# yezhen17/3DIoUMatch

Measured on AMD Instinct MI355X. Metric: scenes/sec train-step (ScanNet 40k pts, 256 proposals), higher is better.
Workload: dtype f32; 1 GPU; ScanNet pretrain step (BASELINE configs[1]): VoteNet-IoU forward_with_pred_jitter + labeled loss + backward + Adam; per_gpu_batch=8, global_batch=8, num_points=40000, num_proposals=256, parallelism=dp1, fps_prefetch_one_step_ahead=True, hip_graphs=True

## Files before the change

3dioumatch_amd/csrc/mlp_gemm.hip:

```cpp
#include "common.h"
#include "mlp_operand.h"
#include <mutex>
#include <stdlib.h>

namespace {

constexpr int KC = 16;

template <int TM, int TN, int WM, int WN, int MODE, bool A_TRANS>
__global__ void __launch_bounds__(256)
gemm_nn_kernel(int m_total, int k_total, int r, const float *__restrict__ a, int lda, OperandB opb,
               float *__restrict__ c, size_t b_stride_in, size_t b_stride_out) {
  constexpr int MB = TM / WM / 32, NB = TN / WN / 32;
  constexpr int LDA = TM + 4;
  __shared__ float As[KC * LDA];
  __shared__ __attribute__((aligned(16))) float Bs[KC * TN];
  const int tid = threadIdx.x, lane = tid & 63, wave = tid >> 6;
  const int wm = wave / WN, wn = wave % WN;
  const int r0 = blockIdx.x * TN, m0 = blockIdx.y * TM, b = blockIdx.z;
  OperandB op = opb;
  const size_t in_off = (size_t)b * b_stride_in;

  f32x16 acc[MB][NB];
#pragma unroll
  for (int i = 0; i < MB; ++i)
#pragma unroll
    for (int j = 0; j < NB; ++j)
#pragma unroll
      for (int q = 0; q < 16; ++q) acc[i][j][q] = 0.f;

  constexpr int AE = TM * KC / 256;
  constexpr int SEG = TN / 16;
  const int bkk = tid >> 4, bnn = (tid & 15) * SEG;
  const bool vec_ok = (r & 3) == 0;
  float areg[AE], bx[SEG], bdz[SEG];
  RowCoef rc;
  bool brow_ok = false;
  auto fetch = [&](int k0) {
#pragma unroll
    for (int e = 0; e < AE; ++e) {
      const int t = tid + e * 256;
      const int kk = A_TRANS ? t / TM : t % KC, mm = A_TRANS ? t % TM : t / KC;
      const int gm = m0 + mm, gk = k0 + kk;
      const size_t at = A_TRANS ? (size_t)gk * lda + gm : (size_t)gm * lda + gk;
      areg[e] = (gm < m_total && gk < k_total) ? a[at] : 0.f;
    }
    const int gk = k0 + bkk;
    brow_ok = gk < k_total;
    rc = load_row_coef<MODE>(op, gk, brow_ok);
    load_raw_segment<MODE, SEG>(op, in_off + (size_t)gk * r + r0 + bnn, r0 + bnn, r, vec_ok,
                                brow_ok, bx, bdz, b * k_total + gk);
  };
  auto stash = [&]() {
#pragma unroll
    for (int e = 0; e < AE; ++e) {
      const int t = tid + e * 256;
      As[(A_TRANS ? t / TM : t % KC) * LDA + (A_TRANS ? t % TM : t / KC)] = areg[e];
    }
#pragma unroll
    for (int i = 0; i < SEG; i += 4) {
      float4 v;
      v.x = (brow_ok && r0 + bnn + i + 0 < r) ? transform<MODE>(bx[i + 0], bdz[i + 0], rc) : 0.f;
      v.y = (brow_ok && r0 + bnn + i + 1 < r) ? transform<MODE>(bx[i + 1], bdz[i + 1], rc) : 0.f;
      v.z = (brow_ok && r0 + bnn + i + 2 < r) ? transform<MODE>(bx[i + 2], bdz[i + 2], rc) : 0.f;
      v.w = (brow_ok && r0 + bnn + i + 3 < r) ? transform<MODE>(bx[i + 3], bdz[i + 3], rc) : 0.f;
      *reinterpret_cast<float4 *>(&Bs[bkk * TN + bnn + i]) = v;
    }
  };
  fetch(0);
  for (int k0 = 0; k0 < k_total; k0 += KC) {
    __syncthreads();
    stash();
    __syncthreads();
    if (k0 + KC < k_total) fetch(k0 + KC);
#pragma unroll
    for (int kk = 0; kk < KC; kk += 2) {
      const int krow = kk + (lane >> 5);
      float af[MB], bf[NB];
#pragma unroll
      for (int i = 0; i < MB; ++i) af[i] = As[krow * LDA + (wm * MB + i) * 32 + (lane & 31)];
#pragma unroll
      for (int j = 0; j < NB; ++j) bf[j] = Bs[krow * TN + (wn * NB + j) * 32 + (lane & 31)];
#pragma unroll
      for (int i = 0; i < MB; ++i)
#pragma unroll
        for (int j = 0; j < NB; ++j)
          acc[i][j] = __builtin_amdgcn_mfma_f32_32x32x2f32(af[i], bf[j], acc[i][j], 0, 0, 0);
    }
// ... 299 lines not shown
    constexpr int GPL = 32 / (PL < 32 ? PL : 32);
#pragma unroll
    for (int i = 0; i < MB; ++i) {
      const int rbase = m0 + (wm * MB + i) * 32;
#pragma unroll
      for (int q = 0; q < 16; ++q) {
        const int cq = (q & 3) + 8 * (q >> 2);
        const int rowq = rbase + cq + 4 * half;
        const bool neg = POOL != 0 && rowq < m_total && pool_gamma[rowq] < 0.f;
        const int rsw = (cq & 15) ^ (half << 2);
#pragma unroll
        for (int j = 0; j < NB; ++j) {
          const int col = j * 32 + l31;
          const float v = acc[i][j][q];
          park[(cq + 4 * half) * 64 + ((((col >> 2) ^ rsw) << 2) | (col & 3))] = neg ? -v : v;
        }
      }
      float best[GPL];
      int at[GPL];
#pragma unroll
      for (int gq = 0; gq < GPL; ++gq) { best[gq] = -__builtin_inff(); at[gq] = 0; }
      const float4 *prow = reinterpret_cast<const float4 *>(park + l31 * 64);
      float t1 = 0.f, t2 = 0.f, tsh = 0.f;
#pragma unroll
      for (int c4 = 0; c4 < 8; ++c4) {
        const float4 v4 = prow[(half * 8 + c4) ^ (l31 & 15)];
        const float vv[4] = {v4.x, v4.y, v4.z, v4.w};
        if (SCAN_STATS && c4 == 0) tsh = vv[0];
#pragma unroll
        for (int e = 0; e < 4; ++e) {
          if constexpr (POOL != 0) {
            const int s2 = c4 * 4 + e;
            const int gq = GPL == 2 ? s2 / 16 : 0;
            if (vv[e] > best[gq]) { best[gq] = vv[e]; at[gq] = GPL == 2 ? s2 % 16 : s2; }
          }
          if constexpr (SCAN_STATS) {
            const float d = vv[e] - tsh;
            t1 += d;
            t2 = __fmaf_rn(d, d, t2);
          }
        }
      }
      if constexpr (SCAN_STATS) {
        const float mh = tsh + t1 * (1.0f / 32.0f), qh = fmaxf(t2 - t1 * t1 * (1.0f / 32.0f), 0.f);
        const float mo = __shfl_xor(mh, 32, kWave), qo = __shfl_xor(qh, 32, kWave);
        if (half == 0) {
          const float dlt = mo - mh;
          float mean = 0.5f * (mh + mo);
          const float m2w = (qh + qo) + 16.0f * dlt * dlt;
          if (POOL != 0 && rbase + l31 < m_total && pool_gamma[rbase + l31] < 0.f) mean = -mean;
          wave_stat[wn][(wm * MB + i) * 32 + l31] = make_float2(mean, m2w);
        }
      }
      if (POOL == 64) {
        const float ob = __shfl_xor(best[0], 32, kWave);
        const int oa = __shfl_xor(at[0], 32, kWave);
        if (half == 0 && ob > best[0]) { best[0] = ob; at[0] = 32 + oa; }
      }
      const int row = rbase + l31;
      if (POOL != 0 && row < m_total && (POOL != 64 || half == 0)) {
        const bool negr = pool_gamma[row] < 0.f;
        const int g0 = (r0 + wn * 64) / POOL + (POOL == 64 ? 0 : half * GPL);
        int *ei = reinterpret_cast<int *>(ext);
#pragma unroll
        for (int gq = 0; gq < GPL; ++gq) {
          const size_t o = ((size_t)b * m_total + row) * groups + g0 + gq;
          ext[o] = negr ? -best[gq] : best[gq];
          ei[ext_plane + o] = at[gq];
        }
      }
    }
    if constexpr (SCAN_STATS) merge_wave_stats();
  }
}

constexpr int KS = 64;

struct AImage {
  const unsigned short *p;
  int pitch;
  size_t plane;
};

template <int MODE, bool A_TRANS, bool X6, bool AIMG = false>
__device__ __forceinline__ void gemm_nn_small_body(int blk_x, int blk_y, int blk_z, int m_total, int k_total,
                                                   int r, const float *__restrict__ a, int lda,
                                                   OperandB opb, float *__restrict__ c,
                                                   size_t b_stride_in, size_t b_stride_out,
                                                   const AImage img = AImage{nullptr, 0, 0}) {
  constexpr int TM = 64, TN = 64, LDA = TM + 1;
  constexpr int STAGE = KS * LDA + KS * TN, REDUCE = 4 * 16 * 64;
  __shared__ __attribute__((aligned(16))) float lds[STAGE > REDUCE ? STAGE : REDUCE];
  float *As = lds + KS * TN, *Bs = lds;
  const int tid = threadIdx.x, lane = tid & 63, wave = tid >> 6;
  const int r0 = blk_x * TN, m0 = blk_y * TM, b = blk_z;
  OperandB op = opb;
  const size_t in_off = (size_t)b * b_stride_in;
  f32x16 acc[2][2];
#pragma unroll
  for (int i = 0; i < 2; ++i)
#pragma unroll
    for (int j = 0; j < 2; ++j)
#pragma unroll
      for (int q = 0; q < 16; ++q) acc[i][j][q] = 0.f;

  const int bkk = tid >> 2, bnn = (tid & 3) * 16;
  const bool vec_ok = (r & 3) == 0;
  float areg[16], bx[16], bdz[16];
  RowCoef rc;
  bool brow_ok = false;
  static_assert(!AIMG || X6, "images feed the bf16 form only");
  const bf16x8 *img8 = reinterpret_cast<const bf16x8 *>(img.p);
  auto fetch = [&](int k0) {
    if constexpr (!AIMG) {
#pragma unroll
      for (int e = 0; e < 16; ++e) {
        const int t = tid + e * 256;
        const int kk = A_TRANS ? t / TM : t % KS, mm = A_TRANS ? t % TM : t / KS;
        const int gm = m0 + mm, gk = k0 + kk;
        const size_t at = A_TRANS ? (size_t)gk * lda + gm : (size_t)gm * lda + gk;
        areg[e] = (gm < m_total && gk < k_total) ? a[at] : 0.f;
      }
    }
    const int gk = k0 + bkk;
    brow_ok = gk < k_total;
    rc = load_row_coef<MODE>(op, gk, brow_ok);
    load_raw_segment<MODE, 16>(op, in_off + (size_t)gk * r + r0 + bnn, r0 + bnn, r, vec_ok,
                               brow_ok, bx, bdz, b * k_total + gk);
  };
  fetch(0);
  for (int k0 = 0; k0 < k_total; k0 += KS) {
    Split3 sa_img[2];
    if constexpr (AIMG) {
      const int k0w = wave * (KS / 4) + 8 * (lane >> 5);
#pragma unroll
      for (int i = 0; i < 2; ++i) {
        const size_t at = ((size_t)(m0 + i * 32 + (lane & 31)) * img.pitch + k0 + k0w) >> 3;
        sa_img[i].hi = img8[at];
        sa_img[i].mid = img8[at + (img.plane >> 3)];
        sa_img[i].lo = img8[at + 2 * (img.plane >> 3)];
      }
    }
    __syncthreads();
    if constexpr (!AIMG) {
#pragma unroll
      for (int e = 0; e < 16; ++e) {
        const int t = tid + e * 256;
        As[(A_TRANS ? t / TM : t % KS) * LDA + (A_TRANS ? t % TM : t / KS)] = areg[e];
      }
    }
#pragma unroll
    for (int i = 0; i < 16; i += 4) {
      float4 v;
      v.x = (brow_ok && r0 + bnn + i + 0 < r) ? transform<MODE>(bx[i + 0], bdz[i + 0], rc) : 0.f;
      v.y = (brow_ok && r0 + bnn + i + 1 < r) ? transform<MODE>(bx[i + 1], bdz[i + 1], rc) : 0.f;
      v.z = (brow_ok && r0 + bnn + i + 2 < r) ? transform<MODE>(bx[i + 2], bdz[i + 2], rc) : 0.f;
      v.w = (brow_ok && r0 + bnn + i + 3 < r) ? transform<MODE>(bx[i + 3], bdz[i + 3], rc) : 0.f;
      *reinterpret_cast<float4 *>(&Bs[bkk * TN + bnn + i]) = v;
    }
    __syncthreads();
    if (k0 + KS < k_total) fetch(k0 + KS);
    if constexpr (X6) {
      static_assert(KS / 4 == 16, "a wave's share of the chunk is one 16-deep MFMA step");
      const int k0w = wave * (KS / 4) + 8 * (lane >> 5);
      Split3 sa[2], sb[2];
      if constexpr (AIMG) {
        sa[0] = sa_img[0]; sa[1] = sa_img[1];
      } else {
#pragma unroll
        for (int i = 0; i < 2; ++i) {
          float v[8];
#pragma unroll
          for (int e = 0; e < 8; ++e) v[e] = As[(k0w + e) * LDA + i * 32 + (lane & 31)];
          sa[i] = split3(v);
        }
      }
#pragma unroll
      for (int j = 0; j < 2; ++j) {
        float v[8];
#pragma unroll
        for (int e = 0; e < 8; ++e) v[e] = Bs[(k0w + e) * TN + j * 32 + (lane & 31)];
        sb[j] = split3(v);
      }
#pragma unroll
      for (int i = 0; i < 2; ++i)
#pragma unroll
        for (int j = 0; j < 2; ++j) mfma_x6(acc[i][j], sa[i], sb[j]);
    } else {
#pragma unroll
    for (int kk = 0; kk < KS / 4; kk += 2) {
      const int krow = wave * (KS / 4) + kk + (lane >> 5);
      float af[2], bf[2];
#pragma unroll
      for (int i = 0; i < 2; ++i) af[i] = As[krow * LDA + i * 32 + (lane & 31)];
#pragma unroll
      for (int j = 0; j < 2; ++j) bf[j] = Bs[krow * TN + j * 32 + (lane & 31)];
#pragma unroll
      for (int i = 0; i < 2; ++i)
#pragma unroll
        for (int j = 0; j < 2; ++j)
          acc[i][j] = __builtin_amdgcn_mfma_f32_32x32x2f32(af[i], bf[j], acc[i][j], 0, 0, 0);
    }
    }
  }
  for (int s = 1; s < 4; ++s) {
    __syncthreads();
    if (wave == s) {
#pragma unroll
      for (int i = 0; i < 2; ++i)
#pragma unroll
        for (int j = 0; j < 2; ++j)
#pragma unroll
          for (int q = 0; q < 16; ++q) lds[((i * 2 + j) * 16 + q) * 64 + lane] = acc[i][j][q];
    }
    __syncthreads();
    if (wave == 0) {
#pragma unroll
      for (int i = 0; i < 2; ++i)
#pragma unroll
        for (int j = 0; j < 2; ++j)
#pragma unroll
          for (int q = 0; q < 16; ++q) acc[i][j][q] += lds[((i * 2 + j) * 16 + q) * 64 + lane];
    }
  }
  if (wave != 0) return;
  float *cb = c + (size_t)b * b_stride_out;
#pragma unroll
  for (int i = 0; i < 2; ++i)
#pragma unroll
    for (int j = 0; j < 2; ++j) {
      const int col = r0 + j * 32 + (lane & 31);
#pragma unroll
      for (int q = 0; q < 16; ++q) {
        const int row = m0 + i * 32 + (q & 3) + 8 * (q >> 2) + 4 * (lane >> 5);
        if (row < m_total && col < r) __builtin_nontemporal_store(acc[i][j][q], &cb[(size_t)row * r + col]);
      }
    }
}

template <int MODE, bool A_TRANS, bool X6 = false, bool AIMG = false>
__global__ void __launch_bounds__(256, (X6 && A_TRANS) ? 2 : 1)
gemm_nn_small_kernel(int m_total, int k_total, int r, const float *__restrict__ a, int lda,
                     OperandB opb, float *__restrict__ c, size_t b_stride_in,
                     size_t b_stride_out, AImage img) {
  gemm_nn_small_body<MODE, A_TRANS, X6, AIMG>((int)blockIdx.x, (int)blockIdx.y, (int)blockIdx.z, m_total,
                                              k_total, r, a, lda, opb, c, b_stride_in, b_stride_out, img);
}

constexpr int RC = 32;

template <int PMODE, int QMODE, int KBW, int WK, int RS>
__global__ void __launch_bounds__(256)
gemm_wgrad_kernel(int m_total, int k_begin, int k_end, int k_total, int r, int r_per_slice,
                  OperandB opp, OperandB opq, float *__restrict__ part, size_t p_stride,
                  size_t q_stride) {
  static_assert(WK * RS == 4, "four waves");
  constexpr int TM = 64, TK = 32 * KBW * WK;
  constexpr int QSEG = TK / 64;
  constexpr int LDP = TM + 1, LDQ = TK + 1;
  constexpr int STAGE = RC * (LDP + LDQ);
  constexpr int REDUCE = RS > 1 ? WK * 2 * KBW * 16 * 64 : 0;
  __shared__ float lds[STAGE > REDUCE ? STAGE : REDUCE];
  float *Ps = lds, *Qs = lds + RC * LDP;
  const int tid = threadIdx.x, lane = tid & 63, wave = tid >> 6;
  const int wk = wave % WK, wr = wave / WK;
  const BlockId blk = xcd_block_id();
  const int k0 = k_begin + blk.x * TK, m0 = blk.y * TM;
  const int slices = (r + r_per_slice - 1) / r_per_slice;
  const int b = blk.z / slices, slice = blk.z % slices;
  const int r_lo = slice * r_per_slice;
  const int r_hi = r_lo + r_per_slice < r ? r_lo + r_per_slice : r;
  OperandB P = opp, Q = opq;
  const size_t p_off = (size_t)b * p_stride, q_off = (size_t)b * q_stride;

  f32x16 acc[2][KBW];
#pragma unroll
  for (int i = 0; i < 2; ++i)
#pragma unroll
    for (int j = 0; j < KBW; ++j)
#pragma unroll
      for (int q = 0; q < 16; ++q) acc[i][j][q] = 0.f;

  const int seg_row = tid >> 2, seg_r = (tid & 3) * 8;
  const bool p_ok = m0 + seg_row < m_total;
  const RowCoef pc = load_row_coef<PMODE>(P, m0 + seg_row, p_ok);
  const size_t p_row = p_off + (size_t)(m0 + seg_row) * r;
  bool q_ok[QSEG];
  RowCoef qc[QSEG];
  size_t q_row[QSEG];
#pragma unroll
  for (int s = 0; s < QSEG; ++s) {
    const int gk = k0 + seg_row + 64 * s;
    q_ok[s] = gk < k_end;
    qc[s] = load_row_coef<QMODE>(Q, gk, q_ok[s]);
    q_row[s] = q_off + (size_t)gk * r;
  }
  const bool vec_ok = ((r | r_hi) & 3) == 0;
  float px[8], pdz[8], qx[QSEG][8], qdz[QSEG][8];
  auto fetch = [&](int rr) {
    load_raw_segment<PMODE, 8>(P, p_row + rr + seg_r, rr + seg_r, r_hi, vec_ok, p_ok, px, pdz,
                               b * m_total + m0 + seg_row);
#pragma unroll
    for (int s = 0; s < QSEG; ++s)
      load_raw_segment<QMODE, 8>(Q, q_row[s] + rr + seg_r, rr + seg_r, r_hi, vec_ok, q_ok[s],
                                 qx[s], qdz[s]);
  };
  fetch(r_lo);
  for (int rr = r_lo; rr < r_hi; rr += RC) {
    __syncthreads();
#pragma unroll
    for (int i = 0; i < 8; ++i)
      Ps[(seg_r + i) * LDP + seg_row] =
          (p_ok && rr + seg_r + i < r_hi) ? transform<PMODE>(px[i], pdz[i], pc) : 0.f;
#pragma unroll
    for (int s = 0; s < QSEG; ++s)
#pragma unroll
      for (int i = 0; i < 8; ++i)
        Qs[(seg_r + i) * LDQ + seg_row + 64 * s] =
            (q_ok[s] && rr + seg_r + i < r_hi) ? transform<QMODE>(qx[s][i], qdz[s][i], qc[s]) : 0.f;
    __syncthreads();
    if (rr + RC < r_hi) fetch(rr + RC);
#pragma unroll
    for (int st = 0; st < RC / 2 / RS; ++st) {
      const int row = wr * (RC / RS) + 2 * st + (lane >> 5);
      float bq[KBW], ap[2];
#pragma unroll
      for (int j = 0; j < KBW; ++j) bq[j] = Qs[row * LDQ + (wk * KBW + j) * 32 + (lane & 31)];
#pragma unroll
// ... 73 lines not shown
    q_ok[i] = gk < k_total;
    pc[i] = load_row_coef<PMODE>(P, gm, p_ok[i]);
    qc[i] = load_row_coef<QMODE>(Q, gk, q_ok[i]);
    p_row[i] = (size_t)b * p_stride + (size_t)gm * r;
    q_row[i] = (size_t)b * q_stride + (size_t)gk * r;
  }
  const bool vec_ok = (r & 3) == 0;
  float px[2][16], pdz[2][16], qx[2][16], qdz[2][16];
  auto fetch = [&](int c0) {
    const int col = c0 + 16 * half;
#pragma unroll
    for (int i = 0; i < 2; ++i) {
      load_raw_segment<PMODE, 16>(P, p_row[i] + col, col, r_hi, vec_ok, p_ok[i], px[i], pdz[i]);
      load_raw_segment<QMODE, 16>(Q, q_row[i] + col, col, r_hi, vec_ok, q_ok[i], qx[i], qdz[i]);
    }
  };
  int c0 = r_lo + 32 * wave;
  if (c0 < r_hi) fetch(c0);
  for (; c0 < r_hi; c0 += 128) {
    const int col = c0 + 16 * half;
#pragma unroll
    for (int st = 0; st < 2; ++st) {
      Split3 sp[2], sq[2];
#pragma unroll
      for (int i = 0; i < 2; ++i) {
        float vp[8], vq[8];
#pragma unroll
        for (int e = 0; e < 8; ++e) {
          const bool in = col + 8 * st + e < r_hi;
          vp[e] = (p_ok[i] && in) ? transform<PMODE>(px[i][8 * st + e], pdz[i][8 * st + e], pc[i]) : 0.f;
          vq[e] = (q_ok[i] && in) ? transform<QMODE>(qx[i][8 * st + e], qdz[i][8 * st + e], qc[i]) : 0.f;
        }
        sp[i] = split3(vp);
        sq[i] = split3(vq);
      }
      if (st == 1 && c0 + 128 < r_hi) fetch(c0 + 128);
#pragma unroll
      for (int i = 0; i < 2; ++i)
#pragma unroll
        for (int j = 0; j < 2; ++j) mfma_x6(acc[i][j], sp[i], sq[j]);
    }
  }
#pragma unroll
  for (int i = 0; i < 2; ++i)
#pragma unroll
    for (int j = 0; j < 2; ++j) {
      __syncthreads();
      if (wave != 0) {
#pragma unroll
        for (int q = 0; q < 16; ++q) red[((wave * 16) + q) * 64 + lane] = acc[i][j][q];
      }
      __syncthreads();
      if (wave == 0) {
#pragma unroll
        for (int q = 0; q < 16; ++q)
          acc[i][j][q] += (red[(16 + q) * 64 + lane] + red[(32 + q) * 64 + lane]) + red[(48 + q) * 64 + lane];
      }
    }
  if (wave != 0) return;
  float *out = part + (size_t)blk.z * m_total * k_total;
#pragma unroll
  for (int i = 0; i < 2; ++i)
#pragma unroll
    for (int j = 0; j < 2; ++j) {
      const int col = k0 + j * 32 + l31;
#pragma unroll
      for (int q = 0; q < 16; ++q) {
        const int row = m0 + i * 32 + (q & 3) + 8 * (q >> 2) + 4 * half;
        if (row < m_total && col < k_total) out[(size_t)row * k_total + col] = acc[i][j][q];
      }
    }
}

template <int PMODE, int QMODE>
__global__ void __launch_bounds__(256, 2)
gemm_wgrad_direct_kernel(int m_total, int k_total, int r, int r_per_slice, int slices, OperandB opp,
                         OperandB opq, float *__restrict__ part, size_t p_stride, size_t q_stride) {
  wgrad_direct_body<PMODE, QMODE>(xcd_block_id(), m_total, k_total, r, r_per_slice, slices, opp, opq,
                                  part, p_stride, q_stride);
}

struct SmallPairArgs {
  int nd, dgx, dgy;
  int m, k, r;
  int wkx, wmy, per, slices;
  const float *w;
  float *dq, *part;
  AImage wt_img;
};

template <int PMODE, int QMODE, bool X6D, bool AIMG = false>
__global__ void __launch_bounds__(256, 2)
gemm_small_backward_pair_kernel(SmallPairArgs t, OperandB opp, OperandB opq) {
  const int id = (int)blockIdx.x;
  if (id < t.nd) {
    const int bx = id % t.dgx, by = (id / t.dgx) % t.dgy, bz = id / (t.dgx * t.dgy);
    gemm_nn_small_body<PMODE, true, X6D, AIMG>(bx, by, bz, t.k, t.m, t.r, t.w, t.k, opp, t.dq,
                                               (size_t)t.m * t.r, (size_t)t.k * t.r, t.wt_img);
  } else {
    const int wid = id - t.nd;
    BlockId blk;
    blk.x = wid % t.wkx;
    blk.y = (wid / t.wkx) % t.wmy;
    blk.z = wid / (t.wkx * t.wmy);
    wgrad_direct_body<PMODE, QMODE>(blk, t.m, t.k, t.r, t.per, t.slices, opp, opq, t.part,
                                    (size_t)t.m * t.r, (size_t)t.k * t.r);
  }
}

template <bool VEC>
__device__ __forceinline__ void reduce_partials_block(int block, int count, int parts,
                                                      const float *__restrict__ part,
                                                      float *__restrict__ out) {
  constexpr int W = VEC ? 4 : 1;
  __shared__ float sums[8][32 * W];
  const int e = threadIdx.x & 31, grp = threadIdx.x >> 5;
  const int i = (block * 32 + e) * W;
  float s[8][W];
#pragma unroll
  for (int u = 0; u < 8; ++u)
#pragma unroll
    for (int c = 0; c < W; ++c) s[u][c] = 0.f;
  auto row = [&](int p, float (&v)[W]) {
    if constexpr (VEC) {
      const float4 t = *reinterpret_cast<const float4 *>(part + (size_t)p * count + i);
      v[0] = t.x; v[1] = t.y; v[2] = t.z; v[3] = t.w;
    } else {
      v[0] = part[(size_t)p * count + i];
    }
  };
  if (i < count) {
    int p = grp;
    for (; p + 56 < parts; p += 64) {
      float v[8][W];
#pragma unroll
      for (int u = 0; u < 8; ++u) row(p + 8 * u, v[u]);
#pragma unroll
      for (int u = 0; u < 8; ++u)
#pragma unroll
        for (int c = 0; c < W; ++c) s[u][c] += v[u][c];
    }
    for (; p + 24 < parts; p += 32) {
      float v[4][W];
#pragma unroll
      for (int u = 0; u < 4; ++u) row(p + 8 * u, v[u]);
#pragma unroll
      for (int u = 0; u < 4; ++u)
#pragma unroll
        for (int c = 0; c < W; ++c) s[u][c] += v[u][c];
    }
    for (; p < parts; p += 8) {
      float v[W];
      row(p, v);
#pragma unroll
      for (int c = 0; c < W; ++c) s[0][c] += v[c];
    }
  }
#pragma unroll
  for (int c = 0; c < W; ++c)
    sums[grp][e * W + c] = ((s[0][c] + s[1][c]) + (s[2][c] + s[3][c])) + ((s[4][c] + s[5][c]) + (s[6][c] + s[7][c]));
  __syncthreads();
  if (grp == 0 && i < count) {
#pragma unroll
    for (int c = 0; c < W; ++c) {
      float t = sums[0][e * W + c];
#pragma unroll
      for (int q = 1; q < 8; ++q) t += sums[q][e * W + c];
      out[i + c] = t;
    }
  }
}

__global__ void __launch_bounds__(256)
reduce_partials_kernel(int count, int parts, const float *__restrict__ part,
                       float *__restrict__ out) {
  reduce_partials_block<false>((int)blockIdx.x, count, parts, part, out);
}

constexpr int kReduceBatch = 40;
struct ReduceBatch {
  int n;
  int first_block[kReduceBatch + 1];
  int count[kReduceBatch];
  int parts[kReduceBatch];
  const float *part[kReduceBatch];
  float *out[kReduceBatch];
  unsigned char vec[kReduceBatch];
};

__global__ void __launch_bounds__(256) reduce_partials_batch_kernel(const ReduceBatch t) {
  const int blk = (int)blockIdx.x;
  int e = 0;
  while (e + 1 < t.n && blk >= t.first_block[e + 1]) ++e;
  if (t.vec[e]) reduce_partials_block<true>(blk - t.first_block[e], t.count[e], t.parts[e], t.part[e], t.out[e]);
  else reduce_partials_block<false>(blk - t.first_block[e], t.count[e], t.parts[e], t.part[e], t.out[e]);
}

template <int TM, int TN, int WM, int WN, int MODE, bool A_TRANS>
void launch_stats(bool a_vec, int r, int b, hipStream_t stream, int rows, int k, const float *a_t,
                  int lda, unsigned a_bytes, const OperandB &op, float *c_t, size_t in_stride,
                  size_t out_stride, float *stats, int channels, int done) {
  if constexpr (!A_TRANS && MODE <= OP_BNRELU) {
    float *st = stats + (size_t)done * 2;
#define ST_LAUNCH(AV)                                                                             \
  hipLaunchKernelGGL((gemm_nn2_kernel<TM, TN, WM, WN, MODE, false, AV, true>),                      \
                     dim3(pn2_ceil_div(r, TN), 1, b), dim3(256), 0, stream, rows, k, r, a_t, lda,   \
                     a_bytes, op, c_t, in_stride, out_stride, st, channels)
    if (a_vec) ST_LAUNCH(true); else ST_LAUNCH(false);
#undef ST_LAUNCH
  }
}

template <int MODE, bool A_TRANS = false>
int launch_nn(int b, int m, int k, int r, const float *a, int lda, const OperandB &op, float *c,
              size_t in_stride, size_t out_stride, hipStream_t stream, float *stats = nullptr,
              const AImage img = AImage{nullptr, 0, 0}) {
  const char *env = getenv("MLP_SMALL_GEMM_COLS");
  const long long small_cols = env ? atoll(env) : 16384;
  if ((long long)b * r <= small_cols) {
    if ((!A_TRANS || MODE == OP_DIRECT) && img.p != nullptr)
      hipLaunchKernelGGL((gemm_nn_small_kernel<MODE, A_TRANS, true, true>),
                         dim3(pn2_ceil_div(r, 64), pn2_ceil_div(m, 64), b), dim3(256), 0, stream, m,
                         k, r, a, lda, op, c, in_stride, out_stride, img);
    else if (!A_TRANS || MODE == OP_DIRECT)
      hipLaunchKernelGGL((gemm_nn_small_kernel<MODE, A_TRANS, true>),
                         dim3(pn2_ceil_div(r, 64), pn2_ceil_div(m, 64), b), dim3(256), 0, stream, m,
                         k, r, a, lda, op, c, in_stride, out_stride, AImage{nullptr, 0, 0});
    else
      hipLaunchKernelGGL((gemm_nn_small_kernel<MODE, A_TRANS>),
                         dim3(pn2_ceil_div(r, 64), pn2_ceil_div(m, 64), b), dim3(256), 0, stream, m,
                         k, r, a, lda, op, c, in_stride, out_stride, AImage{nullptr, 0, 0});
    return pn2_launch_status();
  }
  const bool pipelined = r % 256 == 0;
  const size_t a_total = A_TRANS ? (size_t)k * lda : (size_t)m * lda;
  int done = 0;
  while (done < m) {
    const int left = m - done;
    const float *a_t = A_TRANS ? a + done : a + (size_t)done * lda;
    const unsigned a_bytes = (unsigned)(4 * (A_TRANS ? a_total - done : a_total - (size_t)done * lda));
    float *c_t = c + (size_t)done * r;
    const bool a_vec = (lda & 3) == 0 && (reinterpret_cast<size_t>(a_t) & 15) == 0;
#define NN(TM, TN, WM, WN)                                                                      \
  do {                                                                                          \
    if (stats)                                                                                  \
      launch_stats<TM, TN, WM, WN, MODE, A_TRANS>(a_vec, r, b, stream, rows, k, a_t, lda, a_bytes, \
                                                  op, c_t, in_stride, out_stride, stats, m, done); \
    else if (pipelined && a_vec)                                                                \
      hipLaunchKernelGGL((gemm_nn2_kernel<TM, TN, WM, WN, MODE, A_TRANS, true>),                \
                         dim3(pn2_ceil_div(r, TN), 1, b), dim3(256), 0, stream, rows, k, r, a_t,  \
                         lda, a_bytes, op, c_t, in_stride, out_stride);                         \
    else if (pipelined)                                                                         \
      hipLaunchKernelGGL((gemm_nn2_kernel<TM, TN, WM, WN, MODE, A_TRANS, false>),               \
                         dim3(pn2_ceil_div(r, TN), 1, b), dim3(256), 0, stream, rows, k, r, a_t,  \
                         lda, a_bytes, op, c_t, in_stride, out_stride);                         \
    else                                                                                        \
      hipLaunchKernelGGL((gemm_nn_kernel<TM, TN, WM, WN, MODE, A_TRANS>),                       \
                         dim3(pn2_ceil_div(r, TN), 1, b), dim3(256), 0, stream, rows, k, r, a_t,  \
                         lda, op, c_t, in_stride, out_stride);                                  \
  } while (0)
    int rows;
    if (left >= 256) { rows = 256; NN(256, 64, 4, 1); }
    else if (left > 64) { rows = left < 128 ? left : 128; NN(128, 128, 2, 2); }
    else if (left > 32) { rows = left; NN(64, 128, 2, 2); }
    else {
      rows = left;
      hipLaunchKernelGGL((gemm_nn_kernel<32, 256, 1, 4, MODE, A_TRANS>),
                         dim3(pn2_ceil_div(r, 256), 1, b), dim3(256), 0, stream, rows, k, r, a_t,
                         lda, op, c_t, in_stride, out_stride);
    }
#undef NN
    done += rows;
  }
  return pn2_launch_status();
}

constexpr int kImageBatch = 24;
struct ImageBatch {
  int n;
  int first_tile[kImageBatch + 1];
  int m[kImageBatch], k[kImageBatch];
  const float *w[kImageBatch];
  unsigned short *img[kImageBatch], *img_t[kImageBatch];
};

__host__ __device__ inline int pad64(int v) { return (v + 63) & ~63; }

__global__ void __launch_bounds__(256) weight_images_kernel(const ImageBatch t) {
  __shared__ unsigned short tile[3][64][66];
  int e = 0;
  while (e + 1 < t.n && (int)blockIdx.x >= t.first_tile[e + 1]) ++e;
  const int local = (int)blockIdx.x - t.first_tile[e];
  const int m = t.m[e], k = t.k[e], mp = pad64(m), kp = pad64(k);
  const int tiles_k = kp / 64;
  const int r0 = (local / tiles_k) * 64, c0 = (local % tiles_k) * 64;
  const float *w = t.w[e];
  const size_t plane = (size_t)mp * kp;
  const int tid = threadIdx.x;
  for (int i = tid; i < 64 * 64; i += 256) {
    const int rr = i >> 6, cc = i & 63;
    const float x = (r0 + rr < m && c0 + cc < k) ? w[(size_t)(r0 + rr) * k + c0 + cc] : 0.f;
    const float h = __builtin_bit_cast(float, __builtin_bit_cast(unsigned, x) & 0xffff0000u);
    const float r1 = x - h;
    const float md = __builtin_bit_cast(float, __builtin_bit_cast(unsigned, r1) & 0xffff0000u);
    const float lo = r1 - md;
    tile[0][rr][cc] = (unsigned short)(__builtin_bit_cast(unsigned, h) >> 16);
    tile[1][rr][cc] = (unsigned short)(__builtin_bit_cast(unsigned, md) >> 16);
    tile[2][rr][cc] = (unsigned short)(__builtin_bit_cast(unsigned, lo) >> 16);
  }
  __syncthreads();
  for (int i = tid; i < 3 * 64 * 64; i += 256) {
    const int pl = i >> 12, rr = (i >> 6) & 63, cc = i & 63;
    t.img[e][pl * plane + (size_t)(r0 + rr) * kp + c0 + cc] = tile[pl][rr][cc];
    t.img_t[e][pl * plane + (size_t)(c0 + rr) * mp + r0 + cc] = tile[pl][cc][rr];
// ... 169 lines not shown
  const unsigned a_bytes = (unsigned)(4 * (size_t)m * k);
#define POOLED(TM, TN, WM, WN, NS)                                                                 \
  hipLaunchKernelGGL((gemm_nn2_kernel<TM, TN, WM, WN, OP_BNRELU, false, true, true, NS>),          \
                     dim3(r / TN, 1, b), dim3(256), 0, stream, m, k, r, w, k, a_bytes, op, y,     \
                     in_stride, out_stride, pairs, m, ext, plane, gamma)
  if (m == 256 && ns == 16) POOLED(256, 64, 4, 1, 16);
  else if (m == 256 && ns == 32) POOLED(256, 64, 4, 1, 32);
  else if (m == 256) POOLED(256, 64, 4, 1, 64);
  else if (ns == 16) POOLED(128, 128, 2, 2, 16);
  else if (ns == 32) POOLED(128, 128, 2, 2, 32);
  else POOLED(128, 128, 2, 2, 64);
#undef POOLED
  return pn2_launch_status();
}

MLP_API int mlp_gemm_forward_stats_lin4(int b, int r, const float *w, const float *x4,
                                        const float *w1, const float *scale, const float *shift,
                                        float *y, float *pairs, void *stream_) {
  const int m = 64, k = 64;
  if (b <= 0 || r <= 0) return 0;
  if (!pairs || mlp_gemm_forward_stats_parts(b, m, k, r, nullptr) == 0 ||
      (reinterpret_cast<size_t>(w) & 15) != 0 || (reinterpret_cast<size_t>(w1) & 15) != 0)
    return (int)hipErrorInvalidValue;
  OperandB op = {x4, nullptr, scale, shift, nullptr, nullptr, nullptr, nullptr, 0, 0, w1};
  hipLaunchKernelGGL((gemm_nn2_kernel<64, 128, 2, 2, OP_LIN4, false, true, true>),
                     dim3(r / 128, 1, b), dim3(256), 0, (hipStream_t)stream_, m, k, r, w, k,
                     (unsigned)(4 * (size_t)m * k), op, y, (size_t)4 * r, (size_t)m * r, pairs, m);
  return pn2_launch_status();
}

MLP_API int mlp_gemm_dgrad(int b, int m, int k, int r, const float *wt, int mode, const float *dy,
                           const float *y, const float *dz, const float *scale,
                           const float *shift, const float *mean, const float *invstd,
                           const float *coef, float *dx, void *stream_) {
  if (b <= 0 || m <= 0 || k <= 0 || r <= 0) return 0;
  const size_t in_stride = (size_t)m * r, out_stride = (size_t)k * r;
  if (mode == OP_DIRECT) {
    OperandB op = {dy, nullptr, nullptr, nullptr, nullptr, nullptr, nullptr};
    return launch_nn<OP_DIRECT>(b, k, m, r, wt, m, op, dx, in_stride, out_stride, (hipStream_t)stream_);
  }
  OperandB op = {y, dz, scale, shift, mean, invstd, coef};
  return launch_nn<OP_DY>(b, k, m, r, wt, m, op, dx, in_stride, out_stride, (hipStream_t)stream_);
}

MLP_API int mlp_gemm_dgrad_nt(int b, int m, int k, int r, const float *w, int mode,
                              const float *dy, const float *y, const float *dz,
                              const float *scale, const float *shift, const float *mean,
                              const float *invstd, const float *coef, float *dx, void *stream_) {
  if (b <= 0 || m <= 0 || k <= 0 || r <= 0) return 0;
  const size_t in_stride = (size_t)m * r, out_stride = (size_t)k * r;
  if (mode == OP_DIRECT) {
    OperandB op = {dy, nullptr, nullptr, nullptr, nullptr, nullptr, nullptr};
    return launch_nn<OP_DIRECT, true>(b, k, m, r, w, k, op, dx, in_stride, out_stride,
                                      (hipStream_t)stream_);
  }
  OperandB op = {y, dz, scale, shift, mean, invstd, coef};
  return launch_nn<OP_DY, true>(b, k, m, r, w, k, op, dx, in_stride, out_stride,
                                (hipStream_t)stream_);
}

static bool wgrad_direct_ok(int b, int m, int k, int r, int pmode, int qmode);
static int wgrad_direct_r_per_slice(int b, int m, int k, int r);

MLP_API int mlp_gemm_backward_small_supported(int b, int m, int k, int r, int pmode, int qmode) {
  const char *env = getenv("MLP_SMALL_GEMM_COLS");
  const long long small_cols = env ? atoll(env) : 16384;
  return b > 0 && m > 0 && k > 0 && (long long)b * r <= small_cols &&
         wgrad_direct_ok(b, m, k, r, pmode, qmode);
}

static int backward_small_impl(int b, int m, int k, int r, const float *w, const void *wt_img, int pmode,
                               const float *dy_or_y, const float *dz, const float *scale,
                               const float *shift, const float *mean, const float *invstd,
                               const float *coef, int qmode, const float *x,
                               const float *xscale, const float *xshift, float *dq, float *dw,
                               float *workspace, void *stream_) {
  if (!mlp_gemm_backward_small_supported(b, m, k, r, pmode, qmode)) return (int)hipErrorInvalidValue;
  hipStream_t stream = (hipStream_t)stream_;
  OperandB P = {dy_or_y, dz, scale, shift, mean, invstd, coef};
  if (pmode == OP_DIRECT) P = OperandB{dy_or_y, nullptr, nullptr, nullptr, nullptr, nullptr, nullptr};
  OperandB Q = {x, nullptr, xscale, xshift, nullptr, nullptr, nullptr};
  SmallPairArgs t;
  t.m = m; t.k = k; t.r = r;
  t.dgx = pn2_ceil_div(r, 64); t.dgy = pn2_ceil_div(k, 64);
  t.nd = dq ? t.dgx * t.dgy * b : 0;
  t.per = wgrad_direct_r_per_slice(b, m, k, r);
  t.slices = (r + t.per - 1) / t.per;
  t.wkx = pn2_ceil_div(k, 64); t.wmy = pn2_ceil_div(m, 64);
  t.w = w; t.dq = dq; t.part = workspace;
  t.wt_img = AImage{reinterpret_cast<const unsigned short *>(wt_img), pad64(m), (size_t)pad64(k) * pad64(m)};
  const int nw = t.wkx * t.wmy * b * t.slices;
  const dim3 grid((unsigned)(t.nd + nw));
#define PAIR(PM, QM, X6D)                                                                        \
  hipLaunchKernelGGL((gemm_small_backward_pair_kernel<PM, QM, X6D>), grid, dim3(256), 0, stream, t, P, Q)
  if (pmode == OP_DIRECT && wt_img != nullptr) {
    if (qmode == OP_DIRECT)
      hipLaunchKernelGGL((gemm_small_backward_pair_kernel<OP_DIRECT, OP_DIRECT, true, true>), grid, dim3(256), 0, stream, t, P, Q);
    else
      hipLaunchKernelGGL((gemm_small_backward_pair_kernel<OP_DIRECT, OP_BNRELU, true, true>), grid, dim3(256), 0, stream, t, P, Q);
  }
  else if (pmode == OP_DIRECT && qmode == OP_DIRECT) PAIR(OP_DIRECT, OP_DIRECT, true);
  else if (pmode == OP_DIRECT) PAIR(OP_DIRECT, OP_BNRELU, true);
  else if (qmode == OP_DIRECT) PAIR(OP_DY, OP_DIRECT, false);
  else PAIR(OP_DY, OP_BNRELU, false);
#undef PAIR
  const int rc = pn2_launch_status();
  if (rc) return rc;
  return mlp_reduce_weight_partials(m * k, b * t.slices, workspace, dw, stream);
}

MLP_API int mlp_gemm_backward_small(int b, int m, int k, int r, const float *w, int pmode,
                                    const float *dy_or_y, const float *dz, const float *scale,
                                    const float *shift, const float *mean, const float *invstd,
                                    const float *coef, int qmode, const float *x,
                                    const float *xscale, const float *xshift, float *dq, float *dw,
                                    float *workspace, void *stream_) {
  return backward_small_impl(b, m, k, r, w, nullptr, pmode, dy_or_y, dz, scale, shift, mean, invstd, coef,
                             qmode, x, xscale, xshift, dq, dw, workspace, stream_);
}

MLP_API int mlp_gemm_backward_small_img(int b, int m, int k, int r, const float *w, const void *img_t,
                                        int pmode, const float *dy_or_y, const float *dz,
                                        const float *scale, const float *shift, const float *mean,
                                        const float *invstd, const float *coef, int qmode,
                                        const float *x, const float *xscale, const float *xshift,
                                        float *dq, float *dw, float *workspace, void *stream_) {
  if (!img_t || !mlp_gemm_image_supported(b, r)) return (int)hipErrorInvalidValue;
  return backward_small_impl(b, m, k, r, w, img_t, pmode, dy_or_y, dz, scale, shift, mean, invstd, coef,
                             qmode, x, xscale, xshift, dq, dw, workspace, stream_);
}

MLP_API int mlp_gemm_dgrad_pooled_nt(int b, int m, int k, int groups, int ns, const float *w,
                                     const float *y, const float *dpooled, const int *argmax,
                                     const float *scale, const float *shift, const float *mean,
                                     const float *invstd, const float *coef, float *dx,
                                     void *stream_) {
  if (b <= 0 || m <= 0 || k <= 0 || groups <= 0 || ns <= 0) return 0;
  const int r = groups * ns;
  const size_t in_stride = (size_t)m * r, out_stride = (size_t)k * r;
  OperandB op = {y, dpooled, scale, shift, mean, invstd, coef, argmax, ns, groups};
  return launch_nn<OP_POOLDY, true>(b, k, m, r, w, k, op, dx, in_stride, out_stride,
                                    (hipStream_t)stream_);
}

MLP_API int mlp_gemm_dgrad_pooled(int b, int m, int k, int groups, int ns, const float *wt,
                                  const float *y, const float *dpooled, const int *argmax,
                                  const float *scale, const float *shift, const float *mean,
                                  const float *invstd, const float *coef, float *dx,
                                  void *stream_) {
  if (b <= 0 || m <= 0 || k <= 0 || groups <= 0 || ns <= 0) return 0;
  const int r = groups * ns;
  const size_t in_stride = (size_t)m * r, out_stride = (size_t)k * r;
  OperandB op = {y, dpooled, scale, shift, mean, invstd, coef, argmax, ns, groups};
  return launch_nn<OP_POOLDY>(b, k, m, r, wt, m, op, dx, in_stride, out_stride,
                              (hipStream_t)stream_);
}

static int wgrad_next_tile(int k_left) {
  if (k_left > 192) return 256;
  if (k_left > 128) return 192;
  if (k_left > 64) return 128;
  return 64;
}

static int wgrad_r_per_slice(int b, int m, int k, int r) {
  const long long target = wgrad_next_tile(k) == 192 ? 480 : 720;
  const long long tiles = (long long)pn2_ceil_div(m, 64) * b;
// ... 110 lines not shown
```

Before: 1379 scenes/s.

## Add panel GEMM kernel with double-buffered bf16-split B planes for small GEMMs

Replaces the X6 (split-bf16) path of the small NN GEMM with a new panel kernel. A fragments are held in registers and prefetched per k-step, while B is split into hi/mid/lo bf16 planes once per chunk and stored in double-buffered, swizzled LDS. Row groups of 64 or 128 rows remove the cross-wave LDS reduction, and a buffer-load fast path handles vectorisable B. The aim is to cut redundant splitting, LDS traffic and the reduction stage, at the cost of more registers and a new occupancy hint of 2 blocks per CU.

```diff
diff --git a/3dioumatch_amd/csrc/mlp_gemm.hip b/3dioumatch_amd/csrc/mlp_gemm.hip
--- a/3dioumatch_amd/csrc/mlp_gemm.hip
+++ b/3dioumatch_amd/csrc/mlp_gemm.hip
@@ -2,8 +2,24 @@
 #include "mlp_operand.h"
 #include <mutex>
 #include <stdlib.h>
+#include <type_traits>
+
+typedef int panel_i32x4 __attribute__((ext_vector_type(4)));
+typedef float panel_f32x4 __attribute__((ext_vector_type(4)));
+__device__ panel_f32x4 panel_buffer_load_x4(panel_i32x4 rsrc, int voffset, int soffset, int aux)
+    __asm("llvm.amdgcn.raw.buffer.load.v4f32");
 
 namespace {
+
+__device__ __forceinline__ panel_i32x4 panel_rsrc(const void *p, unsigned bytes) {
+  const unsigned long long a = (unsigned long long)p;
+  panel_i32x4 r;
+  r.x = __builtin_amdgcn_readfirstlane((int)(unsigned)a);
+  r.y = __builtin_amdgcn_readfirstlane((int)((unsigned)(a >> 32) & 0xFFFFu));
+  r.z = __builtin_amdgcn_readfirstlane((int)bytes);
+  r.w = 0x00020000;
+  return r;
+}
 
 constexpr int KC = 16;
 
@@ -469,12 +485,11 @@
   size_t plane;
 };
 
-template <int MODE, bool A_TRANS, bool X6, bool AIMG = false>
+template <int MODE, bool A_TRANS>
 __device__ __forceinline__ void gemm_nn_small_body(int blk_x, int blk_y, int blk_z, int m_total, int k_total,
                                                    int r, const float *__restrict__ a, int lda,
                                                    OperandB opb, float *__restrict__ c,
-                                                   size_t b_stride_in, size_t b_stride_out,
-                                                   const AImage img = AImage{nullptr, 0, 0}) {
+                                                   size_t b_stride_in, size_t b_stride_out) {
   constexpr int TM = 64, TN = 64, LDA = TM + 1;
   constexpr int STAGE = KS * LDA + KS * TN, REDUCE = 4 * 16 * 64;
   __shared__ __attribute__((aligned(16))) float lds[STAGE > REDUCE ? STAGE : REDUCE];
@@ -496,18 +511,14 @@
   float areg[16], bx[16], bdz[16];
   RowCoef rc;
   bool brow_ok = false;
-  static_assert(!AIMG || X6, "images feed the bf16 form only");
-  const bf16x8 *img8 = reinterpret_cast<const bf16x8 *>(img.p);
   auto fetch = [&](int k0) {
-    if constexpr (!AIMG) {
-#pragma unroll
-      for (int e = 0; e < 16; ++e) {
-        const int t = tid + e * 256;
-        const int kk = A_TRANS ? t / TM : t % KS, mm = A_TRANS ? t % TM : t / KS;
-        const int gm = m0 + mm, gk = k0 + kk;
-        const size_t at = A_TRANS ? (size_t)gk * lda + gm : (size_t)gm * lda + gk;
-        areg[e] = (gm < m_total && gk < k_total) ? a[at] : 0.f;
-      }
+#pragma unroll
+    for (int e = 0; e < 16; ++e) {
+      const int t = tid + e * 256;
+      const int kk = A_TRANS ? t / TM : t % KS, mm = A_TRANS ? t % TM : t / KS;
+      const int gm = m0 + mm, gk = k0 + kk;
+      const size_t at = A_TRANS ? (size_t)gk * lda + gm : (size_t)gm * lda + gk;
+      areg[e] = (gm < m_total && gk < k_total) ? a[at] : 0.f;
     }
     const int gk = k0 + bkk;
     brow_ok = gk < k_total;
@@ -517,24 +528,11 @@
   };
   fetch(0);
   for (int k0 = 0; k0 < k_total; k0 += KS) {
-    Split3 sa_img[2];
-    if constexpr (AIMG) {
-      const int k0w = wave * (KS / 4) + 8 * (lane >> 5);
-#pragma unroll
-      for (int i = 0; i < 2; ++i) {
-        const size_t at = ((size_t)(m0 + i * 32 + (lane & 31)) * img.pitch + k0 + k0w) >> 3;
-        sa_img[i].hi = img8[at];
-        sa_img[i].mid = img8[at + (img.plane >> 3)];
-        sa_img[i].lo = img8[at + 2 * (img.plane >> 3)];
-      }
-    }
     __syncthreads();
-    if constexpr (!AIMG) {
-#pragma unroll
-      for (int e = 0; e < 16; ++e) {
-        const int t = tid + e * 256;
-        As[(A_TRANS ? t / TM : t % KS) * LDA + (A_TRANS ? t % TM : t / KS)] = areg[e];
-      }
+#pragma unroll
+    for (int e = 0; e < 16; ++e) {
+      const int t = tid + e * 256;
+      As[(A_TRANS ? t / TM : t % KS) * LDA + (A_TRANS ? t % TM : t / KS)] = areg[e];
     }
 #pragma unroll
     for (int i = 0; i < 16; i += 4) {
@@ -547,33 +545,6 @@
     }
     __syncthreads();
     if (k0 + KS < k_total) fetch(k0 + KS);
-    if constexpr (X6) {
-      static_assert(KS / 4 == 16, "a wave's share of the chunk is one 16-deep MFMA step");
-      const int k0w = wave * (KS / 4) + 8 * (lane >> 5);
-      Split3 sa[2], sb[2];
-      if constexpr (AIMG) {
-        sa[0] = sa_img[0]; sa[1] = sa_img[1];
-      } else {
-#pragma unroll
-        for (int i = 0; i < 2; ++i) {
-          float v[8];
-#pragma unroll
-          for (int e = 0; e < 8; ++e) v[e] = As[(k0w + e) * LDA + i * 32 + (lane & 31)];
-          sa[i] = split3(v);
-        }
-      }
-#pragma unroll
-      for (int j = 0; j < 2; ++j) {
-        float v[8];
-#pragma unroll
-        for (int e = 0; e < 8; ++e) v[e] = Bs[(k0w + e) * TN + j * 32 + (lane & 31)];
-        sb[j] = split3(v);
-      }
-#pragma unroll
-      for (int i = 0; i < 2; ++i)
-#pragma unroll
-        for (int j = 0; j < 2; ++j) mfma_x6(acc[i][j], sa[i], sb[j]);
-    } else {
 #pragma unroll
     for (int kk = 0; kk < KS / 4; kk += 2) {
       const int krow = wave * (KS / 4) + kk + (lane >> 5);
@@ -588,7 +559,6 @@
         for (int j = 0; j < 2; ++j)
           acc[i][j] = __builtin_amdgcn_mfma_f32_32x32x2f32(af[i], bf[j], acc[i][j], 0, 0, 0);
     }
-    }
   }
   for (int s = 1; s < 4; ++s) {
     __syncthreads();
@@ -625,12 +595,203 @@
     }
 }
 
-template <int MODE, bool A_TRANS, bool X6 = false, bool AIMG = false>
-__global__ void __launch_bounds__(256, (X6 && A_TRANS) ? 2 : 1)
+template <int MODE, bool A_TRANS>
+__global__ void __launch_bounds__(256)
 gemm_nn_small_kernel(int m_total, int k_total, int r, const float *__restrict__ a, int lda,
-                     OperandB opb, float *__restrict__ c, size_t b_stride_in,
-                     size_t b_stride_out, AImage img) {
-  gemm_nn_small_body<MODE, A_TRANS, X6, AIMG>((int)blockIdx.x, (int)blockIdx.y, (int)blockIdx.z, m_total,
+                     OperandB opb, float *__restrict__ c, size_t b_stride_in, size_t b_stride_out) {
+  gemm_nn_small_body<MODE, A_TRANS>((int)blockIdx.x, (int)blockIdx.y, (int)blockIdx.z, m_total, k_total, r,
+                                    a, lda, opb, c, b_stride_in, b_stride_out);
+}
+
+constexpr int PANEL_LDS_BYTES = 2 * 3 * 8 * 64 * 16;
+
+__device__ __forceinline__ int p_slot(int n) { return (n & 48) | ((n + (n >> 4)) & 15); }
+
+template <int MODE, bool A_TRANS, bool AIMG, int WR, int RBW>
+__device__ __forceinline__ void gemm_panel_body(void *lds_, int blk_x, int blk_y, int blk_z, int m_total,
+                                                int k_total, int r, const float *__restrict__ a, int lda,
+                                                OperandB opb, float *__restrict__ c, size_t b_stride_in,
+                                                size_t b_stride_out, const AImage img) {
+  constexpr int WC = 4 / WR, CBW = 2 / WC, PW = 64, RG = 32 * WR * RBW;
+  static_assert(WR * WC == 4 && CBW * WC == 2, "four waves over the row and column blocks");
+  bf16x8 *planes = reinterpret_cast<bf16x8 *>(lds_);
+  uint2 *planes8 = reinterpret_cast<uint2 *>(lds_);
+  const int tid = threadIdx.x, lane = tid & 63, l31 = lane & 31, half = lane >> 5;
+  const int wave = __builtin_amdgcn_readfirstlane(tid >> 6);
+  const int wr = wave / WC, wc = wave % WC;
+  const int r0 = blk_x * PW, m0 = blk_y * RG, b = blk_z;
+  OperandB op = opb;
+  const size_t in_off = (size_t)b * b_stride_in;
+  const int chunks = (k_total + KS - 1) / KS;
+
+  f32x16 acc[RBW][CBW];
+#pragma unroll
+  for (int i = 0; i < RBW; ++i)
+#pragma unroll
+    for (int j = 0; j < CBW; ++j)
+#pragma unroll
+      for (int q = 0; q < 16; ++q) acc[i][j][q] = 0.f;
+
+  const int cg = tid & 15, kq = tid >> 4;
+  const int col0 = r0 + 4 * cg;
+  const bool vec_ok = (r & 3) == 0;
+  int st_at[4];
+#pragma unroll
+  for (int i = 0; i < 4; ++i) st_at[i] = (((kq >> 1) * PW) + p_slot(4 * cg + i)) * 2 + (kq & 1);
+  bool active[RBW];
+  int arow[RBW];
+#pragma unroll
+  for (int i = 0; i < RBW; ++i) {
+    const int row0 = m0 + (wr * RBW + i) * 32;
+    active[i] = row0 < m_total;
+    arow[i] = row0 + l31;
+  }
+  const bf16x8 *img8 = reinterpret_cast<const bf16x8 *>(img.p);
+  struct AFrag { Split3 s; float raw[AIMG ? 1 : 8]; };
+  auto load_a = [&](AFrag &f, int i, int k0, int st) {
+    const int gk0 = k0 + 16 * st + 8 * half;
+    if constexpr (AIMG) {
+      const size_t at = ((size_t)(active[i] ? arow[i] : l31) * img.pitch + gk0) >> 3;
+      f.s.hi = img8[at];
+      f.s.mid = img8[at + (img.plane >> 3)];
+      f.s.lo = img8[at + 2 * (img.plane >> 3)];
+    } else {
+      const int gm = arow[i] < m_total ? arow[i] : m_total - 1;
+#pragma unroll
+      for (int e = 0; e < 8; ++e) {
+        const int gk = gk0 + e < k_total ? gk0 + e : k_total - 1;
+        f.raw[e] = a[A_TRANS ? (size_t)gk * lda + gm : (size_t)gm * lda + gk];
+      }
+    }
+  };
+  auto frag_a = [&](const AFrag &f, int i, int k0, int st) {
+    if constexpr (AIMG) {
+      return f.s;
+    } else {
+      const int gk0 = k0 + 16 * st + 8 * half;
+      float v[8];
+#pragma unroll
+      for (int e = 0; e < 8; ++e) v[e] = (arow[i] < m_total && gk0 + e < k_total) ? f.raw[e] : 0.f;
+      return split3(v);
+    }
+  };
+  int b_slot[CBW];
+#pragma unroll
+  for (int j = 0; j < CBW; ++j) b_slot[j] = half * PW + p_slot((wc * CBW + j) * 32 + l31);
+
+  auto run = [&](auto fast_c) {
+    constexpr bool FAST = decltype(fast_c)::value;
+    const panel_i32x4 rsrc_b = panel_rsrc(op.x + in_off, FAST ? (unsigned)((size_t)k_total * r * 4) : 0u);
+    float bx[4][4], bdz[4][4];
+    RowCoef rc[4];
+    auto fetch = [&](int k0) {
+#pragma unroll
+      for (int j = 0; j < 4; ++j) {
+        const int gk = k0 + 4 * kq + j;
+        if constexpr (FAST) {
+          rc[j] = load_row_coef<MODE>(op, gk < k_total ? gk : k_total - 1, true);
+          const panel_f32x4 v = panel_buffer_load_x4(rsrc_b, (gk * r + col0) * 4, 0, 0);
+#pragma unroll
+          for (int i = 0; i < 4; ++i) { bx[j][i] = v[i]; bdz[j][i] = 0.f; }
+        } else {
+          const bool ok = gk < k_total;
+          rc[j] = load_row_coef<MODE>(op, gk, ok);
+          load_raw_segment<MODE, 4>(op, in_off + (size_t)gk * r + col0, col0, r, vec_ok, ok, bx[j], bdz[j],
+                                    b * k_total + gk);
+        }
+      }
+    };
+    auto stage = [&](int buf, int k0) {
+      typedef unsigned u32x4v __attribute__((ext_vector_type(4)));
+#pragma unroll
+      for (int ip = 0; ip < 2; ++ip) {
+        float v[8];
+#pragma unroll
+        for (int e = 0; e < 8; ++e) {
+          const int i = 2 * ip + (e >> 2), j = e & 3;
+          v[e] = (k0 + 4 * kq + j < k_total && col0 + i < r) ? transform<MODE>(bx[j][i], bdz[j][i], rc[j]) : 0.f;
+        }
+        const Split3 s = split3(v);
+        const u32x4v ph = __builtin_bit_cast(u32x4v, s.hi), pm = __builtin_bit_cast(u32x4v, s.mid),
+                     pl = __builtin_bit_cast(u32x4v, s.lo);
+#pragma unroll
+        for (int h = 0; h < 2; ++h) {
+          uint2 *dst = planes8 + (size_t)buf * (3 * 8 * PW * 2) + st_at[2 * ip + h];
+          dst[0 * 8 * PW * 2] = make_uint2(ph[2 * h], ph[2 * h + 1]);
+          dst[1 * 8 * PW * 2] = make_uint2(pm[2 * h], pm[2 * h + 1]);
+          dst[2 * 8 * PW * 2] = make_uint2(pl[2 * h], pl[2 * h + 1]);
+        }
+      }
+    };
+    AFrag af[RBW][4];
+#pragma unroll
+    for (int i = 0; i < RBW; ++i)
+#pragma unroll
+      for (int st = 0; st < 4; ++st) load_a(af[i][st], i, 0, st);
+    fetch(0);
+    stage(0, 0);
+    fetch(KS);
+    __syncthreads();
+    for (int ch = 0; ch < chunks; ++ch) {
+      const int cur = ch & 1;
+      const int k_next = (ch + 1 < chunks ? ch + 1 : ch) * KS;
+      const bf16x8 *pb = planes + (size_t)cur * (3 * 8 * PW);
+#pragma unroll
+      for (int st = 0; st < 4; ++st) {
+        Split3 sb[CBW];
+#pragma unroll
+        for (int j = 0; j < CBW; ++j) {
+          sb[j].hi = pb[0 * 8 * PW + 2 * st * PW + b_slot[j]];
+          sb[j].mid = pb[1 * 8 * PW + 2 * st * PW + b_slot[j]];
+          sb[j].lo = pb[2 * 8 * PW + 2 * st * PW + b_slot[j]];
+        }
+#pragma unroll
+        for (int i = 0; i < RBW; ++i) {
+          if (active[i]) {
+            const Split3 sa = frag_a(af[i][st], i, ch * KS, st);
+#pragma unroll
+            for (int j = 0; j < CBW; ++j) mfma_x6(acc[i][j], sa, sb[j]);
+          }
+          load_a(af[i][st], i, k_next, st);
+        }
+        if (st == 0) {
+          stage(cur ^ 1, (ch + 1) * KS);
+          fetch((ch + 2) * KS);
+        }
+      }
+      __syncthreads();
+    }
+  };
+  if constexpr (MODE <= OP_BNRELU) {
+    if (vec_ok && (size_t)(k_total + 2 * KS) * r < ((size_t)1 << 28)) run(std::true_type{});
+    else run(std::false_type{});
+  } else {
+    run(std::false_type{});
+  }
+  float *cb = c + (size_t)b * b_stride_out;
+#pragma unroll
+  for (int i = 0; i < RBW; ++i)
+    if (active[i]) {
+#pragma unroll
+      for (int j = 0; j < CBW; ++j) {
+        const int col = r0 + (wc * CBW + j) * 32 + l31;
+#pragma unroll
+        for (int q = 0; q < 16; ++q) {
+          const int row = arow[i] - l31 + (q & 3) + 8 * (q >> 2) + 4 * half;
+          if (row < m_total && col < r) __builtin_nontemporal_store(acc[i][j][q], &cb[(size_t)row * r + col]);
+        }
+      }
+    }
+}
+
+inline int panel_row_group(int rows) { return rows > 64 ? 128 : 64; }
+
+template <int MODE, bool A_TRANS, bool AIMG, int WR>
+__global__ void __launch_bounds__(256, 2)
+gemm_panel_kernel(int m_total, int k_total, int r, const float *__restrict__ a, int lda, OperandB opb,
+                  float *__restrict__ c, size_t b_stride_in, size_t b_stride_out, AImage img) {
+  __shared__ __attribute__((aligned(16))) unsigned char lds[PANEL_LDS_BYTES];
+  gemm_panel_body<MODE, A_TRANS, AIMG, WR, 1>(lds, (int)blockIdx.x, (int)blockIdx.y, (int)blockIdx.z, m_total,
                                               k_total, r, a, lda, opb, c, b_stride_in, b_stride_out, img);
 }
 
@@ -870,6 +1031,7 @@
 
 struct SmallPairArgs {
   int nd, dgx, dgy;
+  int dg_rows;
   int m, k, r;
   int wkx, wmy, per, slices;
   const float *w;
@@ -883,8 +1045,18 @@
   const int id = (int)blockIdx.x;
   if (id < t.nd) {
     const int bx = id % t.dgx, by = (id / t.dgx) % t.dgy, bz = id / (t.dgx * t.dgy);
-    gemm_nn_small_body<PMODE, true, X6D, AIMG>(bx, by, bz, t.k, t.m, t.r, t.w, t.k, opp, t.dq,
-                                               (size_t)t.m * t.r, (size_t)t.k * t.r, t.wt_img);
+    if constexpr (X6D) {
+      __shared__ __attribute__((aligned(16))) unsigned char lds[PANEL_LDS_BYTES];
+      if (t.dg_rows == 128)
+        gemm_panel_body<PMODE, true, AIMG, 4, 1>(lds, bx, by, bz, t.k, t.m, t.r, t.w, t.k, opp, t.dq,
+                                                 (size_t)t.m * t.r, (size_t)t.k * t.r, t.wt_img);
+      else
+        gemm_panel_body<PMODE, true, AIMG, 2, 1>(lds, bx, by, bz, t.k, t.m, t.r, t.w, t.k, opp, t.dq,
+                                                 (size_t)t.m * t.r, (size_t)t.k * t.r, t.wt_img);
+    } else {
+      gemm_nn_small_body<PMODE, true>(bx, by, bz, t.k, t.m, t.r, t.w, t.k, opp, t.dq,
+                                      (size_t)t.m * t.r, (size_t)t.k * t.r);
+    }
   } else {
     const int wid = id - t.nd;
     BlockId blk;
@@ -1006,18 +1178,27 @@
   const char *env = getenv("MLP_SMALL_GEMM_COLS");
   const long long small_cols = env ? atoll(env) : 16384;
   if ((long long)b * r <= small_cols) {
-    if ((!A_TRANS || MODE == OP_DIRECT) && img.p != nullptr)
-      hipLaunchKernelGGL((gemm_nn_small_kernel<MODE, A_TRANS, true, true>),
-                         dim3(pn2_ceil_div(r, 64), pn2_ceil_div(m, 64), b), dim3(256), 0, stream, m,
-                         k, r, a, lda, op, c, in_stride, out_stride, img);
-    else if (!A_TRANS || MODE == OP_DIRECT)
-      hipLaunchKernelGGL((gemm_nn_small_kernel<MODE, A_TRANS, true>),
-                         dim3(pn2_ceil_div(r, 64), pn2_ceil_div(m, 64), b), dim3(256), 0, stream, m,
-                         k, r, a, lda, op, c, in_stride, out_stride, AImage{nullptr, 0, 0});
-    else
+    if constexpr (!A_TRANS || MODE == OP_DIRECT) {
+      const int rg = panel_row_group(m);
+      const dim3 grid(pn2_ceil_div(r, 64), pn2_ceil_div(m, rg), b);
+#define PANEL(AIMG, WR)                                                                          \
+  hipLaunchKernelGGL((gemm_panel_kernel<MODE, A_TRANS, AIMG, WR>), grid, dim3(256), 0, stream, m, k, r, \
+                     a, lda, op, c, in_stride, out_stride, img)
+      if (img.p != nullptr) {
+        if constexpr (MODE <= OP_BNRELU) {
+          if (rg == 128) PANEL(true, 4); else PANEL(true, 2);
+        } else {
+          return (int)hipErrorInvalidValue;
+        }
+      } else {
+        if (rg == 128) PANEL(false, 4); else PANEL(false, 2);
+      }
+#undef PANEL
+    } else {
       hipLaunchKernelGGL((gemm_nn_small_kernel<MODE, A_TRANS>),
                          dim3(pn2_ceil_div(r, 64), pn2_ceil_div(m, 64), b), dim3(256), 0, stream, m,
-                         k, r, a, lda, op, c, in_stride, out_stride, AImage{nullptr, 0, 0});
+                         k, r, a, lda, op, c, in_stride, out_stride);
+    }
     return pn2_launch_status();
   }
   const bool pipelined = r % 256 == 0;
@@ -1353,7 +1534,8 @@
   OperandB Q = {x, nullptr, xscale, xshift, nullptr, nullptr, nullptr};
   SmallPairArgs t;
   t.m = m; t.k = k; t.r = r;
-  t.dgx = pn2_ceil_div(r, 64); t.dgy = pn2_ceil_div(k, 64);
+  t.dg_rows = pmode == OP_DIRECT ? panel_row_group(k) : 64;
+  t.dgx = pn2_ceil_div(r, 64); t.dgy = pn2_ceil_div(k, t.dg_rows);
   t.nd = dq ? t.dgx * t.dgy * b : 0;
   t.per = wgrad_direct_r_per_slice(b, m, k, r);
   t.slices = (r + t.per - 1) / t.per;
```

After: 1388 scenes/s (median of 6 runs). About the same (+0.6%).
